# afombravo/2FAST2Q

Measured on AMD Instinct MI355X. Metric: Mreads/sec matched (150 bp, 20 bp feature, m=1), higher is better.
Workload: dtype u64 (2-bit packed bases) / u8 qualities

## Files before the change

2fast2q_amd/csrc/f2q_count_kernels.h:

```cpp
#pragma once

#define F2Q_HIST_MAX 24576u
#define F2Q_HIST_RANGE 38912u

__device__ __forceinline__ unsigned long long wave_sum(unsigned long long v)
{
    for (int o = 32; o > 0; o >>= 1) v += __shfl_down(v, o, 64);
    return v;
}

__device__ __forceinline__ void flush_stats(const Accum &acc, unsigned long long st[5], unsigned long long *lds8,
                                            unsigned long long *slab_row)
{
    const uint32_t lane = threadIdx.x & 63u;
    if (threadIdx.x < 8) lds8[threadIdx.x] = 0;
    __syncthreads();
    for (int k = 0; k < 5; k++) {
        unsigned long long v = wave_sum(st[k]);
        if (lane == 0 && v) atomicAdd(&lds8[k], v);
    }
    __syncthreads();
    if (threadIdx.x < 5) {
        unsigned long long v = lds8[threadIdx.x];
        if (slab_row) gpw(slab_row)[threadIdx.x] = v;
// ... 345 lines not shown
                if (res[j] == R_SLOW) {
                    unsigned long long st2[5] = {0, 0, 0, 0, 0};
                    const Accum acc2 = acc; const PackedBlock pb2 = pb;
                    multi_slow(runp, libp, &acc2, &pb2, tile, 4u * lane + (uint32_t)j, (int)(lv[j] & F2Q_LEN_MASK), st2);
#pragma unroll
                    for (int k = 0; k < 5; k++) st[k] += st2[k];
                    res[j] = R_SKIP;
                } else if (res[j] == R_NEAR) {
                    st[0]++;
                    if (npart[j] == 0u) { res[j] = R_QFAIL; st[4]++; }
                    else if (forced[j]) res[j] = (!do_near || __popc(forced[j]) > run.miss) ? R_NONALIGNED : R_FORCED;
                }
            }
            for (int k = W; k >= 1; k--) {
                bool mine[4]; bool any = false;
#pragma unroll
                for (int j = 0; j < 4; j++) { mine[j] = res[j] == R_NEAR && npart[j] == (uint32_t)k; any |= mine[j]; }
                if (__ballot(any) == 0ull) continue;
                const PackedGroup &pk = lib.mpk[k - 1];
                const PackedPiece ex = pk.exact;
                const uint32_t ib = pk.ib, exm = (1u << ex.bits) - 1u;
                const uint64_t imask = (1ull << ib) - 1ull;
                if (pk.len == 0u) continue;
                uint32_t s[4];
#pragma unroll
                for (int j = 0; j < 4; j++) s[j] = packed_start(key[j], ex.bits);
                while (mine[0] | mine[1] | mine[2] | mine[3]) {
                    uint64_t v0[4], v1[4];
#pragma unroll
                    for (int j = 0; j < 4; j++)
                        if (mine[j]) { const Slot2 pr = packed_pair(ptab, ex.off + s[j]); v0[j] = pr.a; v1[j] = pr.b; }
#pragma unroll
                    for (int j = 0; j < 4; j++) {
                        if (!mine[j]) continue;
                        if (v0[j] == KEY_EMPTY) mine[j] = false;
                        else if ((v0[j] >> ib) == key[j]) { mine[j] = false; res[j] = R_PERFECT; count_hit((uint32_t)(v0[j] & imask)); }
                        else if (v1[j] == KEY_EMPTY) mine[j] = false;
                        else if ((v1[j] >> ib) == key[j]) { mine[j] = false; res[j] = R_PERFECT; count_hit((uint32_t)(v1[j] & imask)); }
                        else s[j] = (s[j] + 2u) & exm;
                    }
                }
            }
            uint32_t npush = 0;
#pragma unroll
            for (int j = 0; j < 4; j++) {
                if (res[j] == R_NEAR) { if (do_near) npush++; else res[j] = R_NONALIGNED; }
                else if (res[j] == R_FORCED) npush++;
                st[1] += (res[j] == R_PERFECT); st[3] += (res[j] == R_NONALIGNED);
            }
            {
                const unsigned long long b0 = __ballot(npush & 1u), b1 = __ballot(npush & 2u), b2 = __ballot(npush & 4u);
                uint32_t at = q_tail + __builtin_amdgcn_mbcnt_hi((uint32_t)(b0 >> 32), __builtin_amdgcn_mbcnt_lo((uint32_t)b0, 0u))
                              + 2u * __builtin_amdgcn_mbcnt_hi((uint32_t)(b1 >> 32), __builtin_amdgcn_mbcnt_lo((uint32_t)b1, 0u))
                              + 4u * __builtin_amdgcn_mbcnt_hi((uint32_t)(b2 >> 32), __builtin_amdgcn_mbcnt_lo((uint32_t)b2, 0u));
                q_tail += (uint32_t)__popcll(b0) + 2u * (uint32_t)__popcll(b1) + 4u * (uint32_t)__popcll(b2);
#pragma unroll
                for (int j = 0; j < 4; j++)
                    if (res[j] == R_NEAR || res[j] == R_FORCED) {
                        queue[at % F2Q_V2_QCAP] = key[j] | ((unsigned long long)(npart[j] - 1u) << 62);
                        qforced[at % F2Q_V2_QCAP] = forced[j];
                        at++;
                    }
            }
        }
        if (do_near) drain(false);
    }
    if (do_near) drain(true);
    __shared__ unsigned long long st_lds[8];
    flush_stats(acc, st, st_lds, acc.stat_slab ? acc.stat_slab + (uint64_t)blockIdx.x * 8u : nullptr);
    if (USE_LDS) {
        __syncthreads();
        auto row = gpw(acc.slab) + (uint64_t)blockIdx.x * nf;
        for (uint32_t i = tid; i < nf; i += F2Q_V2_THREADS) row[i] = hist[i];
    }
}

#define F2Q_LT_THREADS 1024
#define F2Q_LT_WAVES (F2Q_LT_THREADS / 64)

__device__ __forceinline__ U2 lds_u2(const uint32_t *p)
{
    typedef uint32_t v2 __attribute__((ext_vector_type(2)));
    const v2 v = *reinterpret_cast<const v2 *>(p);
    return U2{v.x, v.y};
}

__device__ __forceinline__ uint32_t lt_count_add(uint32_t *cnt, uint32_t slot)
{
    return atomicAdd(&cnt[slot >> 1], 1u << ((slot & 1u) << 4));
}
__device__ __forceinline__ bool lt_count_passed(uint32_t old, uint32_t slot) { return ((old >> ((slot & 1u) << 4)) & 0xFFFFu) == 0x7FFFu; }
__device__ __forceinline__ void lt_count_handoff(uint32_t *cnt, uint32_t slot, const Accum &acc, const LtDesc &lt)
{
    atomicSub(&cnt[slot >> 1], 0x8000u << ((slot & 1u) << 4));
    acc_add(&acc.counts[gp(lt.feat_of)[slot]], 0x8000ull);
}
__device__ __forceinline__ void lt_count(uint32_t *cnt, uint32_t slot, const Accum &acc, const LtDesc &lt)
{
    if (lt_count_passed(lt_count_add(cnt, slot), slot)) lt_count_handoff(cnt, slot, acc, lt);
}

template <int NQ, int NB, bool NEAR, bool A20, bool MW = false>
__global__ __launch_bounds__(F2Q_LT_THREADS) void k_count_fixed4_lds(const RunDev *__restrict__ runp,
                                                                     const LibDev *__restrict__ libp, PackedBlock pb,
                                                                     Accum acc)
{
    extern __shared__ uint32_t lt_smem[];
    constexpr uint32_t NT = NEAR ? 2u : 1u;
    uint32_t *tg = lt_smem;
    uint32_t *cnt = lt_smem + NT * F2Q_LT_SLOTS;
    const RunDev &run = *runp;
    const LibDev &lib = *libp;
    LtDesc lt = lib.lt;
    if (A20) { lt.hb0 = 20u; lt.hb1 = 20u; lt.len = 20u; }
    const uint32_t nf = lib.n_features;
    const uint32_t tid = threadIdx.x, lane = tid & 63u;
    const uint32_t wave = (uint32_t)__builtin_amdgcn_readfirstlane((int)(tid >> 6));
    FixedGeom g = MW ? fixed_geom_at(0, run.n_iter * run.length, run.thr) : fixed_geom(run);
    if (A20) { g.L = 20; g.nq = 5; g.nb = 2; g.sh = 0; g.qm_first = 0x80808080u; g.qm_last = 0x80808080u; g.kmask = (1ull << 40) - 1ull; }
    const int need = g.st + g.L;
    uint32_t w_reads = 0, w_perfect = 0, w_imperfect = 0, w_qfail = 0;
    constexpr int QR = NQ ? NQ : F2Q_MAXQROWS, BR = NB ? NB : F2Q_MAXBROWS;
    constexpr bool PIPE = NQ != 0;

    struct Rows { U4 b[BR], q[QR]; uint32_t len01, len23; };
    const uint64_t q_stride = (uint64_t)pb.wq * F2Q_TILE, b_stride = (uint64_t)pb.wb * F2Q_TILE;
    const auto q_base = gp(pb.qual) + (uint64_t)g.qw0 * F2Q_TILE + 4u * lane;
    const auto b_base = gp(pb.bases) + (uint64_t)g.bw0 * F2Q_TILE + 4u * lane;
    const auto l_base = gp(pb.len) + 4u * lane;
    auto request_tile = [&](Rows &r, uint32_t t) {
        const auto qp = q_base + (uint64_t)t * q_stride;
        const auto bp = b_base + (uint64_t)t * b_stride;
#pragma unroll
        for (int i = 0; i < BR; i++) r.b[i] = ld_u4<true>(bp + (NB ? i : (i < g.nb ? i : g.nb - 1)) * F2Q_TILE);
#pragma unroll
        for (int i = 0; i < QR; i++) r.q[i] = ld_u4<true>(qp + (NQ ? i : (i < g.nq ? i : g.nq - 1)) * F2Q_TILE);
        typedef uint32_t v2 __attribute__((ext_vector_type(2)));
        const v2 lv = __builtin_nontemporal_load((const v2 F2Q_GLOBAL *)(l_base + (uint64_t)t * F2Q_TILE));
        r.len01 = lv.x; r.len23 = lv.y;
    };
    uint32_t pend_old[4] = {0, 0, 0, 0}, pend_slot[4] = {0, 0, 0, 0}, n_pend = 0;
    auto settle = [&]() {
        bool any = false;
#pragma unroll
        for (int k = 0; k < 4; k++)
            if ((uint32_t)k < n_pend) any |= lt_count_passed(pend_old[k], pend_slot[k]);
        if (any) {
#pragma unroll
            for (int k = 0; k < 4; k++)
                if ((uint32_t)k < n_pend && lt_count_passed(pend_old[k], pend_slot[k])) lt_count_handoff(cnt, pend_slot[k], acc, lt);
        }
        n_pend = 0;
    };
    auto decide_tile = [&](const Rows &r) {
        uint32_t bad[4] = {0, 0, 0, 0};
        bool part_fail[4] = {false, false, false, false};
        if (MW && g.add_hi) {
#pragma unroll
            for (int j = 0; j < 4; j++) {
                const int pv = mw_part_verdict(fixed4_failbits(g, r.q, j), run.n_iter, run.length);
                bad[j] = pv == 2 ? 1u : 0u; part_fail[j] = pv == 1;
            }
        } else if (g.add_hi) {
            if (A20) {
#pragma unroll
                for (int i = 0; i < QR; i++) {
#pragma unroll
                    for (int j = 0; j < 4; j++) {
                        const uint32_t w = u4get(r.q[i], j) & 0x7F7F7F7Fu;
                        bad[j] |= (w + g.add_lo) & ~(w + g.add_hi);
                    }
                }
#pragma unroll
                for (int j = 0; j < 4; j++) bad[j] &= 0x80808080u;
            } else {
#pragma unroll
                for (int i = 0; i < QR; i++)
                    if (NQ || i < g.nq) fixed4_qrow(g, i, r.q[i], bad);
            }
        }
        LtProbe0 p[4]; U2 e0[4], e1[4]; uint32_t klo[4], khi[4], forced[4]; bool cand[4];
#pragma unroll
        for (int j = 0; j < 4; j++) {
            const uint32_t l = ((j < 2 ? r.len01 : r.len23) >> (16 * (j & 1))) & 0xFFFFu;
            const bool live = l != F2Q_LEN_SKIP, qf = live && bad[j] != 0u;
            cand[j] = live && !qf && (int)(l & F2Q_LEN_MASK) >= need && !(MW && part_fail[j]);
            w_reads += (uint32_t)__popcll(__ballot(live));
            w_qfail += (uint32_t)__popcll(__ballot(qf));
            forced[j] = 0;
            if ((l & F2Q_LEN_FLAG) && cand[j]) forced[j] = fixed4_flags(g, r.q, j);
            uint64_t key = fixed4_key(g, r.b, j);
            if (MW && lt.mix) { key = mw_mix(key, lt.mix); if (forced[j]) forced[j] = mw_mix_mask(forced[j], lt.mix); }
            p[j] = lt_probe0(lt, key);
            e0[j] = lds_u2(tg + 2u * p[j].b0);
            e1[j] = lds_u2(tg + 2u * p[j].b1);
            klo[j] = (uint32_t)key; khi[j] = lt_rec_hi(key, forced[j]);
        }
        LtExact x[4];
#pragma unroll
        for (int j = 0; j < 4; j++) x[j] = lt_exact_stage(p[j], e0[j], e1[j], cand[j], forced[j]);
        settle();
#pragma unroll
        for (int j = 0; j < 4; j++) {
            pend_old[j] = 0;
            if (x[j].hit) pend_old[j] = lt_count_add(cnt, x[j].slot);
            pend_slot[j] = x[j].slot;
            w_perfect += (uint32_t)__popcll(__ballot(x[j].hit));
        }
        n_pend = 4;
        if (!NEAR) return;
        uint32_t pre[5], pos[4];
        pre[0] = 0;
#pragma unroll
        for (int j = 0; j < 4; j++) {
            const unsigned long long m = __ballot(x[j].batch);
            pos[j] = pre[j] + __builtin_amdgcn_mbcnt_hi((uint32_t)(m >> 32), __builtin_amdgcn_mbcnt_lo((uint32_t)m, 0u));
            pre[j + 1] = pre[j] + (uint32_t)__popcll(m);
        }
        for (uint32_t lo = 0; lo < pre[4]; lo += 64u) {
            const uint32_t at = lo + lane;
            uint32_t rlo = 0, rhi = 0;
#pragma unroll
            for (int j = 0; j < 4; j++) {
                if (!lt_batch_has(pre, j, lo)) continue;
                const bool send = x[j].batch && pos[j] - lo < 64u;
                const int to = (int)(4u * (send ? pos[j] - lo : lt_dump(pre, j, lo)));
                const uint32_t a = (uint32_t)__builtin_amdgcn_ds_permute(to, (int)klo[j]);
                const uint32_t b = (uint32_t)__builtin_amdgcn_ds_permute(to, (int)khi[j]);
                const bool mine = at >= pre[j] && at < pre[j + 1];
                rlo = mine ? a : rlo; rhi = mine ? b : rhi;
            }
            const bool valid = at < pre[4];
            const LtProbe q = lt_probe(lt, lt_rec_key(rlo, rhi));
            U2 e[4];
#pragma unroll
            for (int k = 0; k < 4; k++) e[k] = lds_u2(tg + (uint32_t)(k >> 1) * F2Q_LT_SLOTS + 2u * q.b[k]);
            const LtVerdict v = lt_decide<NEAR>(lt, q, e, lt_rec_forced(rhi), [&](uint32_t bk) { return lds_u2(tg + 2u * bk); });
            settle();
            const LtPred cm = LT_P(valid), perfect = v.perfect & cm, imperfect = v.imperfect & cm;
            pend_old[0] = 0;
            if (LT_TRUE(perfect | imperfect)) pend_old[0] = lt_count_add(cnt, v.slot);
            pend_slot[0] = v.slot;
            n_pend = 1;
            w_perfect += (uint32_t)__popcll(perfect);
            w_imperfect += (uint32_t)__popcll(imperfect);
        }
    };

    const uint32_t stride = gridDim.x * F2Q_LT_WAVES;
    uint32_t tile = blockIdx.x * F2Q_LT_WAVES + wave;
    const uint32_t last = pb.n_tiles - 1u;
    Rows ra, rb;
    if (PIPE && tile < pb.n_tiles) request_tile(ra, tile);
    {
        typedef uint32_t v4 __attribute__((ext_vector_type(4)));
        const v4 F2Q_GLOBAL *src = (const v4 F2Q_GLOBAL *)gp(lt.tags);
        v4 *dst = reinterpret_cast<v4 *>(tg);
        for (uint32_t i = tid; i < NT * F2Q_LT_SLOTS / 4u; i += F2Q_LT_THREADS) dst[i] = src[i];
        for (uint32_t i = tid; i < F2Q_LT_BUCKETS; i += F2Q_LT_THREADS) cnt[i] = 0;
    }
    __syncthreads();
    if (PIPE) {
        if (tile < pb.n_tiles) {
            for (;;) {
                __builtin_amdgcn_sched_barrier(0);
                request_tile(rb, min(tile + stride, last));
                __builtin_amdgcn_sched_barrier(0);
                decide_tile(ra);
                tile += stride;
                if (tile >= pb.n_tiles) break;
                __builtin_amdgcn_sched_barrier(0);
                request_tile(ra, min(tile + stride, last));
                __builtin_amdgcn_sched_barrier(0);
                decide_tile(rb);
                tile += stride;
                if (tile >= pb.n_tiles) break;
            }
        }
    } else {
        for (; tile < pb.n_tiles; tile += stride) { Rows r; request_tile(r, tile); decide_tile(r); }
    }
    settle();
    __syncthreads();
    {
        auto row = gpw(acc.slab) + (uint64_t)blockIdx.x * nf;
        for (uint32_t i = tid; i < nf; i += F2Q_LT_THREADS) {
            const uint32_t s = gp(lt.slot_of)[i];
            row[i] = (cnt[s >> 1] >> ((s & 1u) << 4)) & 0xFFFFu;
        }
    }
    __syncthreads();
    const bool l0 = lane == 0;
    unsigned long long stv[5] = {l0 ? w_reads : 0u, l0 ? w_perfect : 0u, l0 ? w_imperfect : 0u,
                                 l0 ? w_reads - w_perfect - w_imperfect - w_qfail : 0u, l0 ? w_qfail : 0u};
    flush_stats(acc, stv, reinterpret_cast<unsigned long long *>(lt_smem), acc.stat_slab + (uint64_t)blockIdx.x * 8u);
}

__global__ __launch_bounds__(F2Q_V2_THREADS) void k_extract_fixed4(const RunDev *__restrict__ runp, EcDev ec, PackedBlock pb,
                                                                    Accum acc, uint64_t read_base)
{
    const RunDev &run = *runp;
    const uint32_t tid = threadIdx.x, lane = tid & 63u, wave = tid >> 6;
    const FixedGeom g = fixed_geom(run);
    unsigned long long st[5] = {0, 0, 0, 0, 0};
    uint32_t n_new = 0;
    for (uint32_t base = blockIdx.x * F2Q_V2_WAVES; base < pb.n_tiles; base += gridDim.x * F2Q_V2_WAVES) {
        const uint32_t tile = base + wave;
        if (tile >= pb.n_tiles) continue;
        U4 brow[F2Q_MAXBROWS], qrow[F2Q_MAXQROWS];
        const auto qp = gp(pb.qual) + (uint64_t)tile * pb.wq * F2Q_TILE + 4u * lane;
        const auto bp = gp(pb.bases) + (uint64_t)tile * pb.wb * F2Q_TILE + 4u * lane;
#pragma unroll
        for (int r = 0; r < F2Q_MAXBROWS; r++) {
            uint32_t row = (uint32_t)g.bw0 + (uint32_t)(r < g.nb ? r : (g.nb > 0 ? g.nb - 1 : 0));
            row = row < pb.wb ? row : pb.wb - 1u;
            brow[r] = ld_u4<true>(bp + (uint64_t)row * F2Q_TILE);
        }
#pragma unroll
        for (int r = 0; r < F2Q_MAXQROWS; r++) {
            const uint32_t want = (uint32_t)g.qw0 + (uint32_t)(r < g.nq ? r : (g.nq > 0 ? g.nq - 1 : 0));
            const uint32_t row = want < pb.wq ? want : pb.wq - 1u;
            qrow[r] = want < pb.wq ? ld_u4<true>(qp + (uint64_t)row * F2Q_TILE) : U4{0, 0, 0, 0};
        }
        uint32_t len01 = 0, len23 = 0;
        if (pb.len) {
            typedef uint32_t v2 __attribute__((ext_vector_type(2)));
            v2 lv = *(const v2 F2Q_GLOBAL *)(gp(pb.len) + (uint64_t)tile * F2Q_TILE + 4u * lane);
            len01 = lv.x; len23 = lv.y;
        }
        uint32_t bad[4] = {0, 0, 0, 0};
        if (g.add_hi) {
#pragma unroll
            for (int r = 0; r < F2Q_MAXQROWS; r++)
                if (r < g.nq) fixed4_qrow(g, r, qrow[r], bad);
        }
#pragma unroll
        for (int j = 0; j < 4; j++) {
            const uint32_t l = pb.len ? (((j < 2 ? len01 : len23) >> (16 * (j & 1))) & 0xFFFFu) : pb.rmax;
            if (l == F2Q_LEN_SKIP) continue;
            st[0]++;
            if (bad[j]) { st[4]++; continue; }
            const uint64_t slot = (uint64_t)tile * F2Q_TILE + 4u * lane + (uint32_t)j;
            n_new += ec64_insert_word(ec, fixed4_ec_word(g, brow, qrow, j, l), read_base + pb.first_index + (pb.index ? (uint64_t)gp(pb.index)[slot] : slot));
            st[1]++;
        }
    }
    ec64_report_new(ec, n_new);
    __shared__ unsigned long long st_lds[8];
    flush_stats(acc, st, st_lds, nullptr);
}

#define F2Q_AN_THREADS 256
#define F2Q_AN_WAVES (F2Q_AN_THREADS / 64)
#define F2Q_AN_QCAP 512u

__device__ __noinline__ void anchor_slow(const RunDev *run, const LibDev *lib, const EcDev *ec, const Accum *acc,
                                         const PackedBlock *pb, uint32_t tile, uint32_t slot, int r,
                                         unsigned long long read_index, unsigned long long *st, bool lower = false)
{
    uint8_t seq[F2Q_ANCHOR_MAXLEN], qual[F2Q_ANCHOR_MAXLEN];
    const uint32_t nw = pb->planar_nw;
    const auto bp = gp(pb->bases) + (uint64_t)tile * pb->wb * F2Q_TILE + slot;
    const auto qp = gp(pb->qual) + (uint64_t)tile * pb->wq * F2Q_TILE + slot;
    if (r > F2Q_ANCHOR_MAXLEN) r = F2Q_ANCHOR_MAXLEN;
    for (int i = 0; i < r; i++) {
        const uint32_t lo = bp[(uint64_t)(i >> 5) * F2Q_TILE], hi = bp[(uint64_t)(nw + (i >> 5)) * F2Q_TILE];
        seq[i] = (uint8_t)"ACGT"[((lo >> (i & 31)) & 1u) | (((hi >> (i & 31)) & 1u) << 1)];
        qual[i] = (uint8_t)((qp[(uint64_t)planar_qword((uint32_t)i) * F2Q_TILE] >> (8 * planar_qbyte((uint32_t)i))) & 0xFFu);
        if (qual[i] & 0x80u) { seq[i] = lower ? (uint8_t)(seq[i] | 0x20u) : (uint8_t)'N'; qual[i] &= 0x7Fu; }
    }
    general_read<const uint8_t *>(*run, *lib, *ec, *acc, seq, r, qual, r, read_index, st);
}

template <int NW, int KB, bool EC, bool USE_LDS, bool SAMEQ>
__global__ __launch_bounds__(F2Q_AN_THREADS) void k_count_anchor(const RunDev *__restrict__ runp,
                                                                  const LibDev *__restrict__ libp, EcDev ec,
                                                                  PackedBlock pb, Accum acc, uint64_t read_base)
{
    constexpr int NQW = 8 * NW;
    extern __shared__ unsigned long long smem64[];
    unsigned long long *queue = smem64 + (threadIdx.x >> 6) * F2Q_AN_QCAP;
    uint32_t *qforced = reinterpret_cast<uint32_t *>(smem64 + F2Q_AN_WAVES * F2Q_AN_QCAP) + (threadIdx.x >> 6) * F2Q_AN_QCAP;
    uint32_t *hist = reinterpret_cast<uint32_t *>(smem64 + F2Q_AN_WAVES * F2Q_AN_QCAP) + F2Q_AN_WAVES * F2Q_AN_QCAP;
    const RunDev &run = *runp;
    const LibDev &lib = *libp;
    const uint32_t nf = lib.n_features;
    const uint32_t tid = threadIdx.x, lane = tid & 63u;
    if (USE_LDS && !EC) for (uint32_t i = tid; i < nf; i += F2Q_AN_THREADS) hist[i] = 0;
    __syncthreads();
    uint32_t q_head = 0, q_tail = 0;
    const bool do_near = run.miss > 0;
    const int pk_len = (int)lib.pk.len;
    const uint32_t ah_w = phred_add_hi(run.thr), ah_u = phred_add_hi(run.thr_up), ah_d = phred_add_hi(run.thr_down);
    unsigned long long st[5] = {0, 0, 0, 0, 0};
    uint32_t n_new = 0;
#ifdef F2Q_STAMP
    unsigned long long tp[6] = {0, 0, 0, 0, 0, 0}, t0_, t1_;
#define STAMP(i) do { __builtin_amdgcn_sched_barrier(0); t1_ = __builtin_amdgcn_s_memtime(); __builtin_amdgcn_s_waitcnt(0xC07F); tp[i] += t1_ - t0_; t0_ = t1_; __builtin_amdgcn_sched_barrier(0); } while (0)
#else
#define STAMP(i) do {} while (0)
#endif

    auto count_hit = [&](uint32_t idx) {
        if (USE_LDS) atomicAdd(&hist[idx], 1u);
        else acc_add(&acc.counts[idx], 1ull);
    };

    uint32_t nLO[NW], nHI[NW], nQ[NQW], nl = F2Q_LEN_SKIP;
    auto request_tile = [&](uint32_t t) {
        const auto bpn = gp(pb.bases) + (uint64_t)t * pb.wb * F2Q_TILE + tid;
        const auto qpn = gp(pb.qual) + (uint64_t)t * pb.wq * F2Q_TILE + tid;
        nl = pb.len ? gp(pb.len)[(uint64_t)t * F2Q_TILE + tid] : pb.rmax;
#pragma unroll
        for (int w = 0; w < NW; w++) {
            nLO[w] = __builtin_nontemporal_load(bpn + (uint64_t)w * F2Q_TILE);
            nHI[w] = __builtin_nontemporal_load(bpn + (uint64_t)(NW + w) * F2Q_TILE);
        }
#pragma unroll
        for (int i = 0; i < NQW; i++) nQ[i] = __builtin_nontemporal_load(qpn + (uint64_t)i * F2Q_TILE);
    };
    if (blockIdx.x < pb.n_tiles) request_tile(blockIdx.x);
    for (uint32_t tile = blockIdx.x; tile < pb.n_tiles; tile += gridDim.x) {
#ifdef F2Q_STAMP
        __builtin_amdgcn_sched_barrier(0); t0_ = __builtin_amdgcn_s_memtime(); __builtin_amdgcn_s_waitcnt(0xC07F);
#endif
        const uint32_t l = nl;
        uint32_t LO[NW], HI[NW], Q[NQW];
#pragma unroll
        for (int w = 0; w < NW; w++) { LO[w] = nLO[w]; HI[w] = nHI[w]; }
#pragma unroll
        for (int i = 0; i < NQW; i++) Q[i] = nQ[i];
        __builtin_amdgcn_sched_barrier(0);
        if (tile + gridDim.x < pb.n_tiles) request_tile(tile + gridDim.x);
        __builtin_amdgcn_sched_barrier(0);
// ... 935 lines not shown
```

2fast2q_amd/csrc/f2q_device.h:

```cpp
#pragma once
#include <stdint.h>

#ifndef F2Q_HD
#ifdef __HIPCC__
#define F2Q_HD __host__ __device__ __forceinline__
#else
#define F2Q_HD inline
#endif
#endif

#define F2Q_DEV_MAX_ITER 16
#define F2Q_ANCHOR_MAX 128
#define F2Q_MAX_PIECES 8
#define F2Q_REG_MAXLEN 31
#define F2Q_TILE 256
#define F2Q_LEN_SKIP 0xFFFFu
#define F2Q_LEN_FLAG 0x8000u
#define F2Q_LEN_CASE 0x4000u
#define F2Q_LEN_MASK 0x3FFFu

namespace f2q {

#if defined(__HIP_DEVICE_COMPILE__)
#define F2Q_GLOBAL __attribute__((address_space(1)))
// ... 1200 lines not shown
        const bool t1 = k >= 2;
        const bool open = t1 ? (f1 == 0u) : (f0 == 0u);
        const uint32_t ob = t1 ? lt.hb0 : lt.hb1, om = t1 ? m0 : m1, oq = t1 ? q.h0 : q.h1, keep = t1 ? keep0 : keep1;
#pragma unroll
        for (int i = 0; i < 2; i++) {
            const uint32_t w = i ? e[k].y : e[k].x;
            const bool same = (w >> ob) == q.cmp[k];
            const uint32_t d = ham2_32(((w ^ oq) & om) & keep) + nf;
            const bool c = open & same & (d == 1u);
            n += (uint32_t)c;
            hit = c ? (((uint32_t)t1 << 31) | (2u * q.b[k] + (uint32_t)i)) : hit;
            hitw = c ? w : hitw;
        }
    }
    return n;
}
template <class RD>
F2Q_HD uint32_t lt_slot_of_t1(const LtDesc &lt, const LtProbe &q, uint32_t hitw, RD rd)
{
    const uint32_t fh0 = hitw & ((1u << lt.hb0) - 1u);
    uint32_t b0, c0, b1, c1;
    lt_hash(fh0, lt.hb0, lt.hb1, 0, b0, c0); lt_hash(fh0, lt.hb0, lt.hb1, 1, b1, c1);
    const U2 e0 = rd(b0), e1 = rd(b1);
    const uint32_t w0 = lt_tag(c0, q.h1, lt.hb1), w1 = lt_tag(c1, q.h1, lt.hb1);
    const bool a1 = e0.y == w0, hit0 = (e0.x == w0) | a1, b1y = e1.y == w1;
    return hit0 ? 2u * b0 + (uint32_t)a1 : 2u * b1 + (uint32_t)b1y;
}

#if defined(__HIP_DEVICE_COMPILE__)
typedef unsigned long long LtPred;
#define LT_P(c) __ballot(c)
#define LT_TRUE(p) __builtin_amdgcn_inverse_ballot_w64(p)
#define LT_NOT(p) (~(p))
#else
typedef bool LtPred;
#define LT_P(c) (c)
#define LT_TRUE(p) (p)
#define LT_NOT(p) (!(p))
#endif
#define LT_SEL(p, a, b) (LT_TRUE(p) ? (a) : (b))

struct LtSide { uint32_t x, slot; LtPred any, multi, first; };
F2Q_HD LtSide lt_side(uint32_t want0, uint32_t want1, uint32_t limit, uint32_t b0, uint32_t b1, const U2 &e0, const U2 &e1)
{
    const uint32_t x0 = e0.x ^ want0, x1 = e0.y ^ want0, x2 = e1.x ^ want1, x3 = e1.y ^ want1;
    const LtPred s0 = LT_P(x0 < limit), s1 = LT_P(x1 < limit), s2 = LT_P(x2 < limit), s3 = LT_P(x3 < limit);
    LtSide r;
    r.x = LT_SEL(s0, x0, LT_SEL(s1, x1, LT_SEL(s2, x2, x3)));
    r.first = s0 | s1;
    r.any = r.first | s2 | s3;
    r.multi = (s0 & (s1 | s2 | s3)) | (s1 & (s2 | s3)) | (s2 & s3);
    const LtPred odd = (LT_NOT(s0) & s1) | (LT_NOT(r.first) & LT_NOT(s2));
    r.slot = 2u * LT_SEL(r.first, b0, b1) + (LT_TRUE(odd) ? 1u : 0u);
    return r;
}
struct LtVerdict { LtPred perfect, imperfect, via1; uint32_t slot; };
template <bool NEAR, bool T1SLOT = false, class RD>
F2Q_HD LtVerdict lt_decide(const LtDesc &lt, const LtProbe &q, const U2 (&e)[4], uint32_t forced, RD rd0)
{
    const uint32_t w0 = lt_tag(q.cmp[0], q.h1, lt.hb1), w1 = lt_tag(q.cmp[1], q.h1, lt.hb1);
    const LtSide a = lt_side(w0, w1, 1u << lt.hb1, q.b[0], q.b[1], e[0], e[1]);
    LtSide b = a;
    uint32_t w2 = 0, w3 = 0;
    const LtPred unforced = LT_P(forced == 0u);
    LtPred fast = LT_NOT(a.multi);
    if (!NEAR) fast = fast & unforced;
    LtPred perfect = unforced & fast & a.any & LT_P(a.x == 0u), near = perfect & LT_NOT(perfect);
    LtPred through1 = near;
    uint32_t slot = a.slot;
    if (NEAR) {
        w2 = lt_tag(q.cmp[2], q.h0, lt.hb0); w3 = lt_tag(q.cmp[3], q.h0, lt.hb0);
        b = lt_side(w2, w3, 1u << lt.hb0, q.b[2], q.b[3], e[2], e[3]);
        fast = fast & LT_NOT(b.multi);
        perfect = perfect & fast;
        const LtPred c0 = a.any & LT_P(ham2_32(a.x) == 1u), c1 = b.any & LT_P(ham2_32(b.x) == 1u);
        near = unforced & fast & LT_NOT(perfect) & (c0 ^ c1);
        LtPred via1 = near & c1;
#if defined(__HIP_DEVICE_COMPILE__)
        const bool some_forced = LT_NOT(unforced) != 0ull;
#else
        const bool some_forced = forced != 0u;
#endif
        if (some_forced) {
            const uint32_t l0 = lt.hb0 >> 1;
            const uint32_t p = forced ? lt_ctz(forced) : 0u;
            const bool in0 = p < l0;
            const uint32_t keep = ~(3u << (2u * (in0 ? p : p - l0)));
            const uint32_t xs = in0 ? b.x : a.x;
            const LtPred one = LT_P((forced & (forced - 1u)) == 0u);
            const LtPred g = LT_NOT(unforced) & one & fast & LT_P((xs & keep) == 0u) & LT_P(in0 ? LT_TRUE(b.any) : LT_TRUE(a.any));
            near = near | g;
            via1 = via1 | (g & LT_P(in0));
        }
        if (T1SLOT) { slot = LT_SEL(via1, b.slot, slot); through1 = via1; }
        else if (LT_TRUE(via1)) slot = lt_slot_of_t1(lt, q, b.x ^ LT_SEL(b.first, w2, w3), rd0);
    }
    int sres = 0;
    bool sv1 = false;
    if (!LT_TRUE(fast)) {
        sres = R_NONALIGNED;
        const int ex = forced == 0u ? lt_exact(lt, q, e[0], e[1]) : -1;
        if (ex >= 0) { sres = R_PERFECT; slot = (uint32_t)ex; }
#if defined(__HIP_DEVICE_COMPILE__)
        else if (NEAR && __popc(forced) <= 1) {
#else
        else if (NEAR && __builtin_popcount(forced) <= 1) {
#endif
            uint32_t hit = 0, hitw = 0;
            if (lt_near1(lt, q, e, forced, hit, hitw) == 1u) {
                sres = R_IMPERFECT;
                if (T1SLOT) { slot = hit & 0x7FFFFFFFu; sv1 = (hit >> 31) != 0u; }
                else slot = (hit >> 31) ? lt_slot_of_t1(lt, q, hitw, rd0) : (hit & 0x7FFFFFFFu);
            }
        }
    }
    LtVerdict v;
    v.perfect = perfect | LT_P(sres == R_PERFECT);
    v.imperfect = near | LT_P(sres == R_IMPERFECT);
    v.via1 = through1 | LT_P(sv1);
    v.slot = slot;
    return v;
}

struct LtProbe0 { uint32_t b0, b1, w0, w1; };
F2Q_HD LtProbe0 lt_probe0(const LtDesc &lt, uint64_t key)
{
    const uint32_t h0 = (uint32_t)key & ((1u << lt.hb0) - 1u), h1 = (uint32_t)(key >> lt.hb0);
    LtProbe0 p;
    uint32_t c0, c1;
    lt_hash(h0, lt.hb0, lt.hb1, 0, p.b0, c0);
    lt_hash(h0, lt.hb0, lt.hb1, 1, p.b1, c1);
    p.w0 = lt_tag(c0, h1, lt.hb1); p.w1 = lt_tag(c1, h1, lt.hb1);
    return p;
}
struct LtExact { bool hit, batch; uint32_t slot; };
F2Q_HD LtExact lt_exact_stage(const LtProbe0 &p, const U2 &e0, const U2 &e1, bool cand, uint32_t forced)
{
    const bool a0 = e0.x == p.w0, a1 = e0.y == p.w0, b0 = e1.x == p.w1, b1 = e1.y == p.w1;
    LtExact r;
    r.hit = cand && forced == 0u && (a0 | a1 | b0 | b1);
    r.batch = cand && !r.hit;
    r.slot = (a0 | a1) ? 2u * p.b0 + (uint32_t)a1 : 2u * p.b1 + (uint32_t)b1;
    return r;
}
F2Q_HD uint32_t lt_rec_hi(uint64_t key, uint32_t forced) { return (uint32_t)(key >> 32) | (forced << 10); }
F2Q_HD uint64_t lt_rec_key(uint32_t lo, uint32_t hi) { return ((uint64_t)(hi & 0x3FFu) << 32) | lo; }
F2Q_HD uint32_t lt_rec_forced(uint32_t hi) { return hi >> 10; }
F2Q_HD uint32_t lt_dump(const uint32_t (&pre)[5], int j, uint32_t lo)
{
    const uint32_t s = (pre[j] > lo ? pre[j] : lo) - lo, e = pre[j + 1] - lo < 64u ? pre[j + 1] - lo : 64u;
    return e < 64u ? e : (s ? s - 1u : 0u);
}
F2Q_HD bool lt_batch_has(const uint32_t (&pre)[5], int j, uint32_t lo) { return pre[j] < lo + 64u && pre[j + 1] > lo; }

F2Q_HD uint32_t funnel_shr(uint32_t hi, uint32_t lo, int sh)
{
#if defined(__HIP_DEVICE_COMPILE__)
    return __builtin_amdgcn_alignbit(hi, lo, (uint32_t)sh);
#else
    return sh ? ((lo >> sh) | (hi << (32 - sh))) : lo;
#endif
}
F2Q_HD int ctz32(uint32_t x)
{
#if defined(__HIP_DEVICE_COMPILE__)
    return __ffs((int)x) - 1;
#else
    return __builtin_ctz(x);
#endif
}
F2Q_HD uint32_t range_mask32(int lo, int hi)
{
    lo = lo < 0 ? 0 : lo; hi = hi > 32 ? 32 : hi;
    if (hi <= lo) return 0u;
    uint32_t upper = hi >= 32 ? ~0u : ((1u << hi) - 1u);
    return upper & (lo >= 32 ? 0u : (~0u << lo));
}

template <int NW, int KB>
F2Q_HD void anchor_step(const uint32_t (&P)[NW], int j, uint32_t (&cnt)[KB > 0 ? KB : 1][NW], uint32_t (&ovf)[NW])
{
#pragma unroll
    for (int w = 0; w < NW; w++) {
        uint32_t x = funnel_shr(w + 1 < NW ? P[w + 1] : ~0u, P[w], j);
        if (KB == 0) ovf[w] |= x;
        else {
#pragma unroll
            for (int b = 0; b < KB; b++) { uint32_t c = cnt[b][w] & x; cnt[b][w] ^= x; x = c; }
            ovf[w] |= x;
        }
    }
}

template <int NW, int KB>
F2Q_HD void anchor_step2(const uint32_t (&P)[NW], int j1, int j2, uint32_t (&cnt)[KB > 0 ? KB : 1][NW], uint32_t (&ovf)[NW])
{
#pragma unroll
    for (int w = 0; w < NW; w++) {
        const uint32_t up = w + 1 < NW ? P[w + 1] : ~0u;
        const uint32_t x1 = funnel_shr(up, P[w], j1), x2 = funnel_shr(up, P[w], j2);
        if (KB == 0) ovf[w] |= x1 | x2;
        else {
            const uint32_t c0 = cnt[0][w];
#if defined(__HIP_DEVICE_COMPILE__)
            uint32_t x = __builtin_amdgcn_bitop3_b32(c0, x1, x2, 0xE8);
            cnt[0][w] = __builtin_amdgcn_bitop3_b32(c0, x1, x2, 0x96);
#else
            uint32_t x = (c0 & x1) | (c0 & x2) | (x1 & x2);
            cnt[0][w] = c0 ^ x1 ^ x2;
#endif
#pragma unroll
            for (int b = 1; b < KB; b++) { uint32_t c = cnt[b][w] & x; cnt[b][w] ^= x; x = c; }
            ovf[w] |= x;
        }
    }
}
template <int NW, int KB>
F2Q_HD void anchor_steps(const uint32_t (&P)[NW], uint32_t m, uint32_t (&cnt)[KB > 0 ? KB : 1][NW], uint32_t (&ovf)[NW])
{
    while (m & (m - 1u)) {
        const int j1 = ctz32(m); m &= m - 1u;
        const int j2 = ctz32(m); m &= m - 1u;
        anchor_step2<NW, KB>(P, j1, j2, cnt, ovf);
    }
    if (m) anchor_step<NW, KB>(P, ctz32(m), cnt, ovf);
}

template <int NW, int KB>
F2Q_HD void anchor_compare(const uint32_t (&cnt)[KB > 0 ? KB : 1][NW], const uint32_t (&ovf)[NW], int k, uint32_t (&hit)[NW])
{
#pragma unroll
    for (int w = 0; w < NW; w++) {
        uint32_t gt = 0, eq = ~0u;
#pragma unroll
        for (int b = KB - 1; b >= 0; b--) {
            if ((k >> b) & 1) eq &= cnt[b][w];
            else { gt |= eq & cnt[b][w]; eq &= ~cnt[b][w]; }
        }
        hit[w] = ~gt & ~ovf[w];
    }
}

template <int NW, int KBU, int KBD>
F2Q_HD void anchor_hits2p(const RunDev &run, const uint32_t *up_pos, const uint32_t *down_pos,
                          const uint32_t (&LO)[NW], const uint32_t (&HI)[NW], const uint32_t (&FLG)[NW],
                          uint32_t (&hu)[NW], uint32_t (&hd)[NW])
{
    uint32_t cu[KBU > 0 ? KBU : 1][NW], ou[NW], cd[KBD > 0 ? KBD : 1][NW], od[NW];
#pragma unroll
    for (int w = 0; w < NW; w++) {
        ou[w] = 0; od[w] = 0;
#pragma unroll
        for (int b = 0; b < (KBU > 0 ? KBU : 1); b++) cu[b][w] = 0;
#pragma unroll
        for (int b = 0; b < (KBD > 0 ? KBD : 1); b++) cd[b][w] = 0;
    }
#pragma unroll
    for (int c = 0; c < 4; c++) {
        const uint32_t la = (c & 1) ? ~0u : 0u, ha = (c & 2) ? ~0u : 0u;
        uint32_t P[NW];
#pragma unroll
        for (int w = 0; w < NW; w++) P[w] = (LO[w] ^ la) | (HI[w] ^ ha) | FLG[w];
        if (run.has_up) anchor_steps<NW, KBU>(P, up_pos[c], cu, ou);
        if (run.has_down) anchor_steps<NW, KBD>(P, down_pos[c], cd, od);
    }
    anchor_compare<NW, KBU>(cu, ou, run.msu, hu);
    anchor_compare<NW, KBD>(cd, od, run.msd, hd);
}
template <int NW, int KBU, int KBD>
F2Q_HD void anchor_hits2(const RunDev &run, const uint32_t (&LO)[NW], const uint32_t (&HI)[NW], const uint32_t (&FLG)[NW],
                         uint32_t (&hu)[NW], uint32_t (&hd)[NW])
{
    anchor_hits2p<NW, KBU, KBD>(run, run.up_pos, run.down_pos, LO, HI, FLG, hu, hd);
}

template <int NW>
F2Q_HD int first_hit(const uint32_t (&hit)[NW], int from, int to)
{
    int pos = -1;
#pragma unroll
    for (int w = NW - 1; w >= 0; w--) {
        const uint32_t m = hit[w] & range_mask32(from - 32 * w, to + 1 - 32 * w);
        if (m) pos = 32 * w + ctz32(m);
    }
    return pos;
}

template <int NW>
F2Q_HD bool any_in_range(const uint32_t (&F)[NW], int a, int b)
{
    uint32_t acc = 0;
#pragma unroll
    for (int w = 0; w < NW; w++) acc |= F[w] & range_mask32(a - 32 * w, b - 32 * w);
    return acc != 0;
}

template <int NW>
F2Q_HD uint32_t plane_extract(const uint32_t (&P)[NW], int start, int L)
{
    static_assert(NW <= 16, "plane_extract: at most 16 words");
    const uint32_t sh = (uint32_t)start & 31u, wi = (uint32_t)start >> 5;
    constexpr int NV = NW <= 8 ? 8 : 16;
    uint32_t V[NV];
#pragma unroll
    for (int w = 0; w < NV; w++) V[w] = w < NW ? funnel_shr(w + 1 < NW ? P[w + 1] : 0u, P[w], sh) : 0u;
    const bool b0 = wi & 1u, b1 = wi & 2u, b2 = wi & 4u;
// ... 306 lines not shown
```

Before: 175,400.

## Carry partial near-match batches across tiles to keep wave lanes full

Reads that miss the exact lookup and need a near-match probe were compacted per tile and processed in 64-lane batches, with the final partial batch run at low lane occupancy every tile. Now an incomplete batch is carried in registers into the next tile and only full batches are processed, with one masked flush after the tile loop. Each candidate is moved with a single permute per sub-row instead of one per batch iteration. This cuts the number of underfilled lt_probe/lt_decide passes, in exchange for extra register state kept live across tiles and more complex lane-index logic.

```diff
diff --git a/2fast2q_amd/csrc/f2q_count_kernels.h b/2fast2q_amd/csrc/f2q_count_kernels.h
--- a/2fast2q_amd/csrc/f2q_count_kernels.h
+++ b/2fast2q_amd/csrc/f2q_count_kernels.h
@@ -521,6 +521,22 @@
         }
         n_pend = 0;
     };
+    uint32_t rlo = 0, rhi = 0, n_carry = 0;
+    auto decide_batch = [&](LtPred cm) {
+        const LtProbe q = lt_probe(lt, lt_rec_key(rlo, rhi));
+        U2 e[4];
+#pragma unroll
+        for (int k = 0; k < 4; k++) e[k] = lds_u2(tg + (uint32_t)(k >> 1) * F2Q_LT_SLOTS + 2u * q.b[k]);
+        const LtVerdict v = lt_decide<NEAR>(lt, q, e, lt_rec_forced(rhi), [&](uint32_t bk) { return lds_u2(tg + 2u * bk); });
+        settle();
+        const LtPred perfect = v.perfect & cm, imperfect = v.imperfect & cm;
+        pend_old[0] = 0;
+        if (LT_TRUE(perfect | imperfect)) pend_old[0] = lt_count_add(cnt, v.slot);
+        pend_slot[0] = v.slot;
+        n_pend = 1;
+        w_perfect += (uint32_t)__popcll(perfect);
+        w_imperfect += (uint32_t)__popcll(imperfect);
+    };
     auto decide_tile = [&](const Rows &r) {
         uint32_t bad[4] = {0, 0, 0, 0};
         bool part_fail[4] = {false, false, false, false};
@@ -579,41 +595,36 @@
         n_pend = 4;
         if (!NEAR) return;
         uint32_t pre[5], pos[4];
-        pre[0] = 0;
+        pre[0] = n_carry;
 #pragma unroll
         for (int j = 0; j < 4; j++) {
             const unsigned long long m = __ballot(x[j].batch);
             pos[j] = pre[j] + __builtin_amdgcn_mbcnt_hi((uint32_t)(m >> 32), __builtin_amdgcn_mbcnt_lo((uint32_t)m, 0u));
             pre[j + 1] = pre[j] + (uint32_t)__popcll(m);
         }
-        for (uint32_t lo = 0; lo < pre[4]; lo += 64u) {
+        uint32_t a[4], b[4];
+#pragma unroll
+        for (int j = 0; j < 4; j++) {
+            a[j] = 0; b[j] = 0;
+            if (pre[j] == pre[j + 1]) continue;
+            const int to = (int)(4u * lt_carry_to(pre, j, x[j].batch, pos[j]));
+            a[j] = (uint32_t)__builtin_amdgcn_ds_permute(to, (int)klo[j]);
+            b[j] = (uint32_t)__builtin_amdgcn_ds_permute(to, (int)khi[j]);
+        }
+        uint32_t lo = 0;
+        for (;;) {
             const uint32_t at = lo + lane;
-            uint32_t rlo = 0, rhi = 0;
 #pragma unroll
             for (int j = 0; j < 4; j++) {
-                if (!lt_batch_has(pre, j, lo)) continue;
-                const bool send = x[j].batch && pos[j] - lo < 64u;
-                const int to = (int)(4u * (send ? pos[j] - lo : lt_dump(pre, j, lo)));
-                const uint32_t a = (uint32_t)__builtin_amdgcn_ds_permute(to, (int)klo[j]);
-                const uint32_t b = (uint32_t)__builtin_amdgcn_ds_permute(to, (int)khi[j]);
-                const bool mine = at >= pre[j] && at < pre[j + 1];
-                rlo = mine ? a : rlo; rhi = mine ? b : rhi;
-            }
-            const bool valid = at < pre[4];
-            const LtProbe q = lt_probe(lt, lt_rec_key(rlo, rhi));
-            U2 e[4];
-#pragma unroll
-            for (int k = 0; k < 4; k++) e[k] = lds_u2(tg + (uint32_t)(k >> 1) * F2Q_LT_SLOTS + 2u * q.b[k]);
-            const LtVerdict v = lt_decide<NEAR>(lt, q, e, lt_rec_forced(rhi), [&](uint32_t bk) { return lds_u2(tg + 2u * bk); });
-            settle();
-            const LtPred cm = LT_P(valid), perfect = v.perfect & cm, imperfect = v.imperfect & cm;
-            pend_old[0] = 0;
-            if (LT_TRUE(perfect | imperfect)) pend_old[0] = lt_count_add(cnt, v.slot);
-            pend_slot[0] = v.slot;
-            n_pend = 1;
-            w_perfect += (uint32_t)__popcll(perfect);
-            w_imperfect += (uint32_t)__popcll(imperfect);
-        }
+                if (!lt_carry_has(pre, j, lo)) continue;
+                const bool mine = lt_carry_take(pre, j, at);
+                rlo = mine ? a[j] : rlo; rhi = mine ? b[j] : rhi;
+            }
+            if (pre[4] - lo < 64u) break;
+            decide_batch(LT_P(true));
+            lo += 64u;
+        }
+        n_carry = pre[4] - lo;
     };
 
     const uint32_t stride = gridDim.x * F2Q_LT_WAVES;
@@ -649,6 +660,7 @@
     } else {
         for (; tile < pb.n_tiles; tile += stride) { Rows r; request_tile(r, tile); decide_tile(r); }
     }
+    if (NEAR && n_carry) decide_batch(__ballot(lane < n_carry));
     settle();
     __syncthreads();
     {
diff --git a/2fast2q_amd/csrc/f2q_device.h b/2fast2q_amd/csrc/f2q_device.h
--- a/2fast2q_amd/csrc/f2q_device.h
+++ b/2fast2q_amd/csrc/f2q_device.h
@@ -1376,6 +1376,9 @@
     return e < 64u ? e : (s ? s - 1u : 0u);
 }
 F2Q_HD bool lt_batch_has(const uint32_t (&pre)[5], int j, uint32_t lo) { return pre[j] < lo + 64u && pre[j + 1] > lo; }
+F2Q_HD uint32_t lt_carry_to(const uint32_t (&pre)[5], int j, bool send, uint32_t pos) { return (send ? pos : pre[j + 1]) & 63u; }
+F2Q_HD bool lt_carry_has(const uint32_t (&pre)[5], int j, uint32_t lo) { return pre[j] < pre[j + 1] && lt_batch_has(pre, j, lo); }
+F2Q_HD bool lt_carry_take(const uint32_t (&pre)[5], int j, uint32_t at) { return at >= pre[j] && at < pre[j + 1]; }
 
 F2Q_HD uint32_t funnel_shr(uint32_t hi, uint32_t lo, int sh)
 {
```

After: 176,400, median of 6. No clear change (+0.5%).
